# facebookresearch/momentum

Hardware: NVIDIA H100
Metric: GN iterations/sec (batched 72-joint IK) (higher is better)
Workload: dtype f32

## Files before the change

### momentum_b200/csrc/ik_chol_sched.cpp

```cpp
#include "ik_chol_sched.h"

#include "ik_chol_sched.cuh"

#include <algorithm>
#include <cstdio>
#include <cstdlib>
#include <map>
#include <set>
#include <tuple>

namespace mb2 {

namespace {

struct BitRows {
  int n, words;
  std::vector<uint64_t> b;
  BitRows(int n_) : n(n_), words((n_ + 63) / 64), b(size_t(n_) * ((n_ + 63) / 64), 0) {}
  uint64_t* row(int i) { return b.data() + size_t(i) * words; }
  const uint64_t* row(int i) const { return b.data() + size_t(i) * words; }
  void set(int i, int j) { row(i)[j >> 6] |= 1ull << (j & 63); }
  void clear(int i, int j) { row(i)[j >> 6] &= ~(1ull << (j & 63)); }
  bool test(int i, int j) const { return (row(i)[j >> 6] >> (j & 63)) & 1ull; }
  int count(int i) const {
    int c = 0;
    for (int w = 0; w < words; ++w) c += __builtin_popcountll(row(i)[w]);
    return c;
  }
};

std::vector<int> minimumDegreeOrder(BitRows& adj, const std::vector<int>* priority) {
  const int n = adj.n;
  std::vector<int> order;
  order.reserve(n);
  std::vector<uint8_t> done(n, 0);
  std::vector<int> degree(n);
  for (int i = 0; i < n; ++i) degree[i] = adj.count(i);
  int last = -1;
  for (int step = 0; step < n; ++step) {
    int best = -1;
    for (int i = 0; i < n; ++i) {
      if (done[i]) continue;
      if (best < 0 || degree[i] < degree[best]) { best = i; continue; }
      if (degree[i] != degree[best]) continue;
      const int pi = priority ? (*priority)[i] : 0, pb = priority ? (*priority)[best] : 0;
      if (pi > pb) best = i;
      else if (pi == pb && last >= 0 && adj.test(last, i) && !adj.test(last, best)) best = i;
    }
    std::vector<int> nb;
    for (int j = 0; j < n; ++j)
      if (!done[j] && j != best && adj.test(best, j)) nb.push_back(j);
    for (int u : nb) {
      uint64_t* ru = adj.row(u);
      const uint64_t* rv = adj.row(best);
      for (int w = 0; w < adj.words; ++w) ru[w] |= rv[w];
      adj.clear(u, u);
      adj.clear(u, best);
    }
    for (int u : nb) {
      int c = 0;
      for (int j : nb) c += (j != u) ? 1 : 0;
      (void)c;
      int d = 0;
      const uint64_t* ru = adj.row(u);
      for (int j = 0; j < n; ++j)
        if (!done[j] && j != best && ((ru[j >> 6] >> (j & 63)) & 1ull)) ++d;
      degree[u] = d;
    }
    done[best] = 1;
    order.push_back(best);
    last = best;
  }
  return order;
}

}

std::string buildCholSchedule(int n, const std::vector<std::vector<int>>& cliques, bool forceDense, CholSchedule& out, const std::vector<int>* priority) {
  out = CholSchedule();
  if (n <= 0) return "empty system";
  out.n = n;
  out.nParams = n;

  std::vector<int> order(n);
  BitRows pattern(n);
  for (int i = 0; i < n; ++i) pattern.set(i, i);
  if (forceDense) {
    for (int i = 0; i < n; ++i) order[i] = i;
  } else {
    for (const auto& c : cliques)
      for (int a : c) {
        if (a < 0 || a >= n) continue;
        for (int b : c)
          if (b >= 0 && b < n) pattern.set(a, b);
      }
    BitRows work = pattern;
    for (int i = 0; i < n; ++i) work.clear(i, i);
    if (priority != nullptr && int(priority->size()) != n) return "priority must have one entry per column";
    order = minimumDegreeOrder(work, priority);
  }
  std::vector<int> slot(n);
  {
    std::vector<int> rank(n);
    for (int i = 0; i < n; ++i) rank[order[i]] = i;
    BitRows F(n);
    for (int a = 0; a < n; ++a)
      for (int b = 0; b < n; ++b)
        if (a != b && (forceDense || pattern.test(a, b))) { const int i = rank[a], j = rank[b]; if (i > j) F.set(i, j); }
    std::vector<int> parent(n, -1), cnt(n, 0);
    std::vector<std::vector<int>> col(n);
    for (int j = 0; j < n; ++j) {
      for (int i = j + 1; i < n; ++i) if (F.test(i, j)) col[j].push_back(i);
      cnt[j] = int(col[j].size());
      if (!col[j].empty()) {
        const int pj = col[j][0];
        parent[j] = pj;
        for (size_t k = 1; k < col[j].size(); ++k) F.set(col[j][k], pj);
      }
    }
    int fill = 0, start = 0;
    int padded = 0;
    auto closeTile = [&]() { if (fill != 0) { padded += kCholTile - fill; fill = 0; } };
    auto flushSupernode = [&](int first, int lastExcl) {
      const int sz = lastExcl - first;
      if (sz <= kCholTile) {
        if (fill + sz > kCholTile) closeTile();
      } else {
        closeTile();
        const int head = sz % kCholTile;
        for (int j = first; j < first + head; ++j) { slot[j] = padded++; fill = (fill + 1) % kCholTile; }
        closeTile();
        first += head;
      }
      for (int j = first; j < lastExcl; ++j) { slot[j] = padded++; fill = (fill + 1) % kCholTile; }
    };
    for (int j = 1; j <= n; ++j) {
      const bool joins = j < n && parent[j - 1] == j && cnt[j - 1] == cnt[j] + 1;
      if (!joins) { flushSupernode(start, j); start = j; }
    }
    (void)fill;
    const int T0 = (padded + kCholTile - 1) / kCholTile;
    out.numTileCols = T0;
    out.nPad = T0 * kCholTile;
  }
  const int T = out.numTileCols;
  if (T > 512) return "system too large for the tile schedule";
  out.perm.assign(out.nPad, int16_t(-1));
  std::vector<int> pos(n);
  for (int i = 0; i < n; ++i) { out.perm[slot[i]] = int16_t(order[i]); pos[order[i]] = slot[i]; }

  std::vector<std::vector<uint8_t>> S(T, std::vector<uint8_t>(T, 0));
  for (int I = 0; I < T; ++I) S[I][I] = 1;
  if (forceDense) {
    for (int I = 0; I < T; ++I) for (int J = 0; J <= I; ++J) S[I][J] = 1;
  } else {
    for (int a = 0; a < n; ++a)
      for (int b = 0; b < n; ++b)
        if (pattern.test(a, b)) {
          const int I = pos[a] / kCholTile, J = pos[b] / kCholTile;
// ... 77 lines not shown
    start.assign(1, 0);
    for (int L = 0; L < numLevels; ++L) {
      std::vector<int> ids;
      for (int t = out.levelTaskStart[L]; t < out.levelTaskStart[L + 1]; ++t) ids.push_back(t);
      std::stable_sort(ids.begin(), ids.end(), [&](int a, int b) { return out.taskPairStart[a + 1] - out.taskPairStart[a] > out.taskPairStart[b + 1] - out.taskPairStart[b]; });
      std::vector<std::vector<int>> ofWarp(W);
      std::vector<int64_t> load(W, 0);
      for (int t : ids) {
        int w = 0;
        for (int k = 1; k < W; ++k) if (load[k] < load[w]) w = k;
        ofWarp[w].push_back(t);
        load[w] += 2 * (out.taskPairStart[t + 1] - out.taskPairStart[t]) + 1;
      }
      size_t rounds = 0;
      for (const auto& v : ofWarp) rounds = std::max(rounds, v.size());
      const size_t base = order.size();
      order.resize(base + rounds * W, -1);
      for (int w = 0; w < W; ++w)
        for (size_t r = 0; r < ofWarp[w].size(); ++r) order[base + r * W + w] = ofWarp[w][r];
      start.push_back(int32_t(order.size()));
    }
  }
  out.colPanelStart.assign(1, 0);
  for (int K = 0; K < T; ++K) {
    for (int I : st[K]) { out.colPanelTile.push_back(tileId[I][K]); out.colPanelRow.push_back(I); }
    out.colPanelStart.push_back(int(out.colPanelTile.size()));
  }
  for (int K = 0; K < T; ++K) { const int64_t r = T - 1 - K; out.denseTileOps += r * (r + 1) / 2; }
  out.order = order;
  if (getenv("MB2_SCHED_DUMP") != nullptr) {
    fprintf(stderr, "chol schedule: n %d nPad %d tile columns %d tiles %d levels %d tile ops %lld (dense %lld)\n", n, out.nPad, T, out.numTiles, numLevels, (long long)out.tileOps, (long long)out.denseTileOps);
    for (int L = 0; L < numLevels; ++L) {
      int maxPairs = 0, pairs = 0;
      for (int t = out.levelTaskStart[L]; t < out.levelTaskStart[L + 1]; ++t) { const int p = out.taskPairStart[t + 1] - out.taskPairStart[t]; pairs += p; maxPairs = std::max(maxPairs, p); }
      fprintf(stderr, "  level %d: %d diagonal tiles, %d panel tiles, %d update tasks (%d pairs, longest %d), %d vector tasks; columns:", L, out.levelColStart[L + 1] - out.levelColStart[L],
              out.levelPanelStart[L + 1] - out.levelPanelStart[L], out.levelTaskStart[L + 1] - out.levelTaskStart[L], pairs, maxPairs, out.levelVTaskStart[L + 1] - out.levelVTaskStart[L]);
      for (int ci = out.levelColStart[L]; ci < out.levelColStart[L + 1]; ++ci) fprintf(stderr, " %d(%d)", out.levelCols[ci], int(st[out.levelCols[ci]].size()));
      fprintf(stderr, "\n");
    }
  }
  return "";
}

std::string buildGramPlan(const CholSchedule& s, const std::vector<int32_t>& cellRow0, const std::vector<int32_t>& cellRows, const std::vector<int32_t>& cellCol,
                          int numRows, GramPlan& out) {
  out = GramPlan();
  out.numTiles = s.numTiles;
  out.numTileCols = s.numTileCols;
  const int T = s.numTileCols;
  std::map<std::pair<int, int>, int> stripId;
  for (size_t i = 0; i < cellCol.size(); ++i) {
    const int d = cellCol[i];
    if (d < 0 || d >= s.n || s.pos[d] < 0) return "Jacobian cell in a column outside the schedule";
    const int K = s.pos[d] >> 4;
    for (int q = cellRow0[i] >> 2; q <= (cellRow0[i] + cellRows[i] - 1) >> 2; ++q) stripId[{q, K}] = 0;
  }
  int next = 0;
  for (auto& kv : stripId) kv.second = next++;
  out.numStrips = next;
  out.stripCoord.resize(size_t(next) * 2);
  std::vector<std::vector<int>> ofCol(T);
  for (const auto& kv : stripId) {
    const int q = kv.first.first, K = kv.first.second;
    out.stripCoord[2 * kv.second] = 4 * q;
    out.stripCoord[2 * kv.second + 1] = s.perm[16 * K];
    ofCol[K].push_back(kv.second);
  }
  std::map<int, std::set<int>> colsOfUnit;
  std::map<int, int> rowsOfUnit;
  for (size_t i = 0; i < cellCol.size(); ++i) { colsOfUnit[cellRow0[i]].insert(s.pos[cellCol[i]] >> 4); rowsOfUnit[cellRow0[i]] = cellRows[i]; }
  std::set<std::tuple<int, int, int>> quadPairs;
  for (const auto& kv : colsOfUnit) {
    const int r0 = kv.first, r1 = r0 + rowsOfUnit[r0] - 1;
    for (int q = r0 >> 2; q <= r1 >> 2; ++q)
      for (int I : kv.second)
        for (int J : kv.second)
          if (I >= J) quadPairs.insert(std::make_tuple(q, I, J));
  }
  std::vector<std::vector<std::pair<int, int>>> pairs(s.numTiles);
  for (const auto& qp : quadPairs) {
    const int q = std::get<0>(qp), I = std::get<1>(qp), J = std::get<2>(qp);
    const int t = s.tileIdTable[size_t(I) * T + J];
    if (t < 0) return "Gram plan: a Jacobian row couples two tile columns whose tile is not in the schedule";
    pairs[t].push_back({stripId[{q, I}], stripId[{q, J}]});
  }
  out.residOff = out.numStrips * 64;
  out.stride = (out.residOff + ((numRows + 3) & ~3) + 63) / 64 * 64;
  const int zeroStrip = out.stride / 64;
  out.tilePairStart.assign(s.numTiles + 1, 0);
  for (int t = 0; t < s.numTiles; ++t) {
    out.macs += int64_t(pairs[t].size()) * 16 * 16 * 4;
    if (pairs[t].size() % 2) pairs[t].push_back({zeroStrip, zeroStrip});
    out.tilePairStart[t + 1] = out.tilePairStart[t] + int(pairs[t].size());
    for (const auto& pr : pairs[t]) { out.pairA.push_back(pr.first); out.pairB.push_back(pr.second); }
  }
  out.tileQuadStart.assign(s.numTiles + 1, 0);
  for (int t = 0; t < s.numTiles; ++t) {
    out.tileQuadStart[t + 1] = out.tileQuadStart[t] + (out.tilePairStart[t + 1] - out.tilePairStart[t]) / 2;
    for (int p = out.tilePairStart[t]; p < out.tilePairStart[t + 1]; p += 2) {
      out.quad.push_back(out.pairA[p] * 64); out.quad.push_back(out.pairB[p] * 64);
      out.quad.push_back(out.pairA[p + 1] * 64); out.quad.push_back(out.pairB[p + 1] * 64);
    }
  }
  {
    std::vector<int> byLoad(s.numTiles);
    for (int t = 0; t < s.numTiles; ++t) byLoad[t] = t;
    std::stable_sort(byLoad.begin(), byLoad.end(), [&](int a, int b) { return pairs[a].size() > pairs[b].size(); });
    std::vector<std::vector<int>> ofWarp(kGramWarps);
    std::vector<int64_t> load(kGramWarps, 0);
    for (int t : byLoad) {
      int w = 0;
      for (int k = 1; k < kGramWarps; ++k) if (load[k] < load[w]) w = k;
      ofWarp[w].push_back(t);
      load[w] += int64_t(pairs[t].size()) / 2 + 2;
    }
    size_t rounds = 0;
    for (const auto& v : ofWarp) rounds = std::max(rounds, v.size());
    out.tileOrder.assign(rounds * kGramWarps, -1);
    for (int w = 0; w < kGramWarps; ++w)
      for (size_t r = 0; r < ofWarp[w].size(); ++r) out.tileOrder[r * kGramWarps + w] = ofWarp[w][r];
  }
  std::map<int, int> stripsOfQuad;
  for (const auto& kv : stripId) ++stripsOfQuad[kv.first.first];
  out.cellStripOff.resize(cellCol.size());
  out.cellQuadStride.resize(cellCol.size());
  for (size_t i = 0; i < cellCol.size(); ++i) {
    const int d = cellCol[i], K = s.pos[d] >> 4, q0 = cellRow0[i] >> 2;
    out.cellStripOff[i] = uint32_t(stripId[{q0, K}]) * 64u + uint32_t(d - s.perm[16 * K]) * 4u;
    out.cellQuadStride[i] = uint16_t(stripsOfQuad[q0]);
    for (int q = q0 + 1; q <= (cellRow0[i] + cellRows[i] - 1) >> 2; ++q)
      if (stripsOfQuad[q] != stripsOfQuad[q0] || stripId[{q, K}] != stripId[{q0, K}] + (q - q0) * stripsOfQuad[q0]) return "Gram plan: row quads of one unit are not laid out uniformly";
  }
  out.colStripStart.assign(T + 1, 0);
  for (int K = 0; K < T; ++K) {
    out.colStripStart[K + 1] = out.colStripStart[K] + int(ofCol[K].size());
    out.colStrip.insert(out.colStrip.end(), ofCol[K].begin(), ofCol[K].end());
  }
  return "";
}

void makeGramBlob(const GramPlan& g, const CholSchedule& s, std::vector<int32_t>& blob, int32_t offsets[8]) {
  blob.clear();
  int k = 0;
  auto add = [&](const std::vector<int32_t>& v) { offsets[k++] = int32_t(blob.size()); blob.insert(blob.end(), v.begin(), v.end()); while (blob.size() % 4) blob.push_back(0); };
  add(g.tileOrder); add(g.tileQuadStart); add(g.quad); add(std::vector<int32_t>()); add(g.colStripStart); add(g.colStrip);
  std::vector<int32_t> stripRow(g.numStrips), info(s.numTiles);
  for (int i = 0; i < g.numStrips; ++i) stripRow[i] = g.stripCoord[2 * i];
  auto validOf = [&](int K) { int v = 0; while (v < kCholTile && s.perm[16 * K + v] >= 0) ++v; return v; };
  for (int t = 0; t < s.numTiles; ++t) info[t] = validOf(s.tileRow[t]) | (validOf(s.tileCol[t]) << 8) | ((s.tileRow[t] == s.tileCol[t] ? 1 : 0) << 16);
  add(stripRow); add(info);
  if (blob.empty()) blob.push_back(0);
}

std::string makeGramCholTables(const GramPlan& g, const CholSchedule& s, GramCholTables& out) {
  out = GramCholTables();
  std::vector<uint16_t>& t = out.tab;
  bool fits = true;
  auto put = [&](int64_t v) { fits = fits && v >= 0 && v <= 0xFFFF; t.push_back(uint16_t(v)); };
  auto section = [&]() { while (t.size() % 4) t.push_back(0); return int32_t(t.size()); };
  auto validOf = [&](int K) { int v = 0; while (v < kCholTile && s.perm[16 * K + v] >= 0) ++v; return v; };
  out.L.gram = section();
  for (int32_t tile : g.tileOrder) {
    if (tile < 0) { put(0xFFFF); put(0); put(0); put(0); continue; }
    fits = fits && tile < 0xFFFF;
    put(tile);
    put(validOf(s.tileRow[tile]) | (validOf(s.tileCol[tile]) << 8) | ((s.tileRow[tile] == s.tileCol[tile] ? 1 : 0) << 15));
    put(g.tileQuadStart[tile]); put(g.tileQuadStart[tile + 1]);
  }
  out.L.quad = section();
  for (int32_t v : g.quad) put(v);
  out.L.col = section();
  for (int32_t v : g.colStripStart) put(v);
  out.L.colEnt = section();
  for (int32_t sidx : g.colStrip) { put(int64_t(sidx) * 64); put(g.stripCoord[2 * sidx]); }
  out.L.level = section();
  for (int L = 0; L <= s.numLevels; ++L) { put(s.levelColStart[L]); put(s.levelPanelStart[L]); put(s.levelOrderStart8[L]); put(s.levelVTaskStart[L]); }
  out.L.diag = section();
  for (int32_t K : s.levelCols) { put(K); put(s.diagTile[K]); put(s.colPanelStart[K]); put(s.colPanelStart[K + 1]); }
  out.L.panel = section();
  for (size_t pi = 0; pi < s.panelTile.size(); ++pi) { put(s.panelTile[pi]); put(s.panelDiag[pi]); }
  out.L.order = section();
  for (int32_t ti : s.taskOrder8) {
    if (ti < 0) { put(0xFFFF); put(0); put(0); put(0); continue; }
    fits = fits && s.taskDst[ti] < 0xFFFF;
    put(s.taskDst[ti]); put(s.taskPairStart[ti]); put(s.taskPairStart[ti + 1]); put(0);
  }
  out.L.pair = section();
  for (size_t p = 0; p < s.pairA.size(); ++p) { put(s.pairA[p]); put(s.pairB[p]); }
  out.L.vtask = section();
  for (size_t vi = 0; vi < s.vtaskRow.size(); ++vi) { put(s.vtaskRow[vi]); put(s.vtaskSrcStart[vi]); put(s.vtaskSrcStart[vi + 1]); put(0); }
  out.L.vsrc = section();
  for (size_t p = 0; p < s.vsrcTile.size(); ++p) { put(s.vsrcTile[p]); put(s.vsrcCol[p]); }
  out.L.colPanel = section();
  for (size_t p = 0; p < s.colPanelTile.size(); ++p) { put(s.colPanelTile[p]); put(s.colPanelRow[p]); }
  section();
  const int64_t onStrips = (int64_t(g.stride) + 64 + 255) / 256;
  out.parkTiles = int32_t(std::min<int64_t>(s.numTiles, onStrips));
  return fits ? "" : "Gram + Cholesky tables: an entry does not fit in 16 bits";
}

void layoutDeviceColumns(CholSchedule& s, std::vector<int32_t>& deviceColumnOrder) {
  deviceColumnOrder.clear();
  s.nParams = s.n;
  for (int K = 0; K < s.numTileCols; ++K) {
    while (deviceColumnOrder.size() % 4 != 0) deviceColumnOrder.push_back(-1);
    for (int j = 0; j < kCholTile; ++j) {
      int16_t& p = s.perm[16 * K + j];
      if (p < 0) continue;
      const int dev = int(deviceColumnOrder.size());
      deviceColumnOrder.push_back(p);
      p = int16_t(dev);
    }
  }
  s.n = int32_t(deviceColumnOrder.size());
  s.pos.assign(s.n, int16_t(-1));
  for (int slot = 0; slot < s.nPad; ++slot) if (s.perm[slot] >= 0) s.pos[s.perm[slot]] = int16_t(slot);
  s.order.assign(deviceColumnOrder.begin(), deviceColumnOrder.end());
}

}

namespace mb2 {

void makeScheduleBlob(const CholSchedule& s, std::vector<int32_t>& blob, CholSchedDev& dev) {
  blob.clear();
  std::vector<size_t> offs;
  auto add16 = [&](const std::vector<int16_t>& v) { offs.push_back(blob.size()); for (int16_t x : v) blob.push_back(int32_t(x)); while (blob.size() % 4) blob.push_back(0); };
  auto add32 = [&](const std::vector<int32_t>& v) { offs.push_back(blob.size()); blob.insert(blob.end(), v.begin(), v.end()); while (blob.size() % 4) blob.push_back(0); };
  add16(s.perm); add16(s.pos); add16(s.tileIdTable); add16(s.tileRow); add16(s.tileCol);
  add32(s.diagTile); add32(s.levelColStart); add32(s.levelCols); add32(s.levelPanelStart); add32(s.panelTile); add32(s.panelDiag);
  add32(s.levelTaskStart); add32(s.taskDst); add32(s.taskPairStart); add32(s.pairA); add32(s.pairB); add32(s.levelVTaskStart); add32(s.vtaskRow);
  add32(s.vtaskSrcStart); add32(s.vsrcTile); add32(s.vsrcCol); add32(s.colPanelStart); add32(s.colPanelTile); add32(s.colPanelRow);
  add32(s.levelOrderStart8); add32(s.taskOrder8); add32(s.levelOrderStart16); add32(s.taskOrder16);
  {
    std::vector<int32_t> info(size_t(s.numTiles) * 3, 0);
    auto validOf = [&](int K) { int v = 0; while (v < kCholTile && s.perm[16 * K + v] >= 0) ++v; return v; };
    for (int t = 0; t < s.numTiles; ++t) {
      const int I = s.tileRow[t], J = s.tileCol[t];
      const int vI = validOf(I), vJ = validOf(J);
      info[3 * t] = vI > 0 ? s.perm[16 * I] : 0;
      info[3 * t + 1] = vJ > 0 ? s.perm[16 * J] : 0;
      info[3 * t + 2] = vI | (vJ << 8) | ((I == J ? 1 : 0) << 16);
    }
    add32(info);
  }
  if (blob.empty()) blob.push_back(0);
  dev = CholSchedDev();
  dev.n = s.n; dev.nPad = s.nPad; dev.numTileCols = s.numTileCols; dev.numTiles = s.numTiles; dev.numLevels = s.numLevels;
  const int32_t* b = blob.data();
  dev.blob = b;
  dev.blobInts = int32_t(blob.size());
  int k = 0;
  dev.perm = b + offs[k++]; dev.pos = b + offs[k++]; dev.tileIdTable = b + offs[k++]; dev.tileRow = b + offs[k++]; dev.tileCol = b + offs[k++];
  dev.diagTile = b + offs[k++]; dev.levelColStart = b + offs[k++]; dev.levelCols = b + offs[k++]; dev.levelPanelStart = b + offs[k++];
  dev.panelTile = b + offs[k++]; dev.panelDiag = b + offs[k++]; dev.levelTaskStart = b + offs[k++]; dev.taskDst = b + offs[k++];
  dev.taskPairStart = b + offs[k++]; dev.pairA = b + offs[k++]; dev.pairB = b + offs[k++]; dev.levelVTaskStart = b + offs[k++]; dev.vtaskRow = b + offs[k++];
  dev.vtaskSrcStart = b + offs[k++]; dev.vsrcTile = b + offs[k++]; dev.vsrcCol = b + offs[k++]; dev.colPanelStart = b + offs[k++];
  dev.colPanelTile = b + offs[k++]; dev.colPanelRow = b + offs[k++];
  dev.levelOrderStart8 = b + offs[k++]; dev.taskOrder8 = b + offs[k++]; dev.levelOrderStart16 = b + offs[k++]; dev.taskOrder16 = b + offs[k++];
  dev.tileInfo = b + offs[k++];
}

}
```

### momentum_b200/csrc/ik_chol_sched.h

```cpp
#pragma once

#include <cstdint>
#include <string>
#include <vector>

namespace mb2 {

constexpr int kCholTile = 16;

struct CholSchedule {
  int32_t n{0}, nPad{0}, numTileCols{0}, numTiles{0}, numLevels{0};
  int32_t nParams{0};
  std::vector<int16_t> perm;
  std::vector<int16_t> pos;
  std::vector<int16_t> tileIdTable;
  std::vector<int16_t> tileRow, tileCol;
  std::vector<int32_t> diagTile;
  std::vector<int32_t> levelColStart, levelCols;
  std::vector<int32_t> levelPanelStart, panelTile, panelDiag, panelRow;
  std::vector<int32_t> levelTaskStart, taskDst, taskPairStart, pairA, pairB;
  std::vector<int32_t> levelOrderStart8, taskOrder8, levelOrderStart16, taskOrder16;
  std::vector<int32_t> levelVTaskStart, vtaskRow, vtaskSrcStart, vsrcTile, vsrcCol;
  std::vector<int32_t> colPanelStart, colPanelTile, colPanelRow;
  std::vector<int> order;
  int64_t tileOps{0};
  int64_t denseTileOps{0};
};

std::string buildCholSchedule(int n, const std::vector<std::vector<int>>& cliques, bool forceDense, CholSchedule& out, const std::vector<int>* priority = nullptr);
void layoutDeviceColumns(CholSchedule& s, std::vector<int32_t>& deviceColumnOrder);

inline int cholSchedLdH(int n) { return (n + 1 + 15) / 16 * 16; }
constexpr int kGramWarps = 8;
constexpr int kGramCholMaxRounds = 8;
struct GramPlan {
  int32_t numStrips{0}, numTiles{0}, numTileCols{0};
  std::vector<int32_t> stripCoord;
  std::vector<int32_t> tileOrder;
  std::vector<int32_t> tilePairStart;
  std::vector<int32_t> pairA, pairB;
  std::vector<int32_t> tileQuadStart;
  std::vector<int32_t> quad;
  std::vector<int32_t> colStripStart;
  std::vector<int32_t> colStrip;
  std::vector<uint32_t> cellStripOff;
  std::vector<uint16_t> cellQuadStride;
  int32_t residOff{0};
  int32_t stride{0};
  int64_t macs{0};
};
std::string buildGramPlan(const CholSchedule& s, const std::vector<int32_t>& cellRow0, const std::vector<int32_t>& cellRows, const std::vector<int32_t>& cellCol,
                          int numRows, GramPlan& out);

void makeGramBlob(const GramPlan& g, const CholSchedule& s, std::vector<int32_t>& blob, int32_t offsets[8]);

struct CholSchedDev;
void makeScheduleBlob(const CholSchedule& s, std::vector<int32_t>& blob, CholSchedDev& dev);

struct GramCholLayout {
  int32_t gram, quad, col, colEnt, level, diag, panel, order, pair, vtask, vsrc, colPanel;
};
struct GramCholTables {
  GramCholLayout L{};
  std::vector<uint16_t> tab;
  int32_t parkTiles{0};
};
std::string makeGramCholTables(const GramPlan& g, const CholSchedule& s, GramCholTables& out);

}
```

### momentum_b200/csrc/ik_kernels.cu

```cuda
#include "ik_kernels.cuh"

#include <algorithm>
#include <cstdio>
#include <type_traits>

#include "ik_chol.cuh"
#include "ik_chol_sched.h"
#include "ik_jtj_tc.cuh"
#include "ik_ptx.cuh"
#include "ik_device.cuh"
#include "ik_jacobi.cuh"

namespace mb2 {

__device__ __forceinline__ double warpSum(double v) {
  for (int o = 16; o > 0; o >>= 1) v += __shfl_xor_sync(0xffffffffu, v, o);
  return v;
}

size_t sweepSmemPerInstance(const FunctionTables& T, int warpsPerInstance) {
  const size_t nPad = (T.numParams + 3) & ~3;
  const size_t jp = warpsPerInstance > 1 ? size_t((T.numJoints * kParametersPerJoint + 1) & ~1) : 0;
  return sizeof(float) * (nPad + jp + size_t((T.numJoints * kJointStateStride + 1) & ~1) + size_t((T.recStride + 1) & ~1) + 4 + 2 * size_t(warpsPerInstance));
}
// ... 1889 lines not shown
        bulkLoad(smemAddr(tiles) + off, reinterpret_cast<const char*>(src) + off, total - off < 16384u ? total - off : 16384u, barAddr);
    }
  } else {
    if (tid == 0) {
      bulkLoad(smemAddr(blob), Sg.blob, blobBytes, barAddr);
      bulkLoad(smemAddr(gsub), a.g + size_t(b) * a.ldG, gBytes, barAddr);
    }
    for (int t = tid; t < Sg.numTiles; t += kSchedThreads) {
      const int gi0 = __ldg(Sg.tileInfo + 3 * t), gj0 = __ldg(Sg.tileInfo + 3 * t + 1);
      tmaLoad3d(smemAddr(tiles + size_t(t) * 256), &hmap, gi0, gj0, b, barAddr);
    }
  }
  MB2_PROF(6)
  mbarWaitRelaxed(barAddr, 0);
  MB2_PROF(7)
  const CholSchedDev S = rebaseSchedule(Sg, blob);
  if (fromGram) {
    for (int s = tid; s < S.nPad; s += kSchedThreads) {
      const int p = S.perm[s];
      if (p >= 0) gsub[p] = y[s];
    }
  } else {
    for (int t = warp; t < S.numTiles; t += kSchedThreads / 32) cholConvertBox(tiles + size_t(t) * 256, S.tileInfo[3 * t + 2], lane);
    for (int s = tid; s < S.nPad; s += kSchedThreads) {
      const int p = S.perm[s];
      y[s] = p >= 0 ? gsub[p] : 0.f;
    }
  }
  __syncthreads();
  MB2_PROF(8)
  if (!fromGram)
    for (int s = tid; s < S.nPad; s += kSchedThreads)
      if (S.perm[s] >= 0) tiles[size_t(S.diagTile[s >> 4]) * 256 + tileIdx(s & 15, s & 15)] += a.regularization;
  __syncthreads();
  MB2_PROF(0)

  for (int L = 0; L < S.numLevels; ++L) {
    for (int ci = S.levelColStart[L] + warp; ci < S.levelColStart[L + 1]; ci += kSchedThreads / 32) {
      const int K = S.levelCols[ci];
      cholDiagTile(tiles + size_t(S.diagTile[K]) * 256, y + 16 * K, lane, a.regularization, flags);
    }
    __syncthreads();
    MB2_PROF(1)
    for (int pi = S.levelPanelStart[L] + warp; pi < S.levelPanelStart[L + 1]; pi += kSchedThreads / 32) {
      float* ptile = tiles + size_t(S.panelTile[pi]) * 256;
      float x[2][4];
      cholPanelProduct(ptile, tiles + size_t(S.panelDiag[pi]) * 256, lane, x);
      cholPanelStore(ptile, lane, x);
    }
    __syncthreads();
    MB2_PROF(2)
    {
      const int32_t* oStart = kSchedThreads == 256 ? S.levelOrderStart8 : S.levelOrderStart16, *order = kSchedThreads == 256 ? S.taskOrder8 : S.taskOrder16;
      for (int oi = oStart[L] + warp; oi < oStart[L + 1]; oi += kSchedThreads / 32) { const int ti = order[oi]; if (ti >= 0) cholUpdateTask(tiles, S, ti, lane); }
    }
    for (int vi = S.levelVTaskStart[L] + hw; vi < S.levelVTaskStart[L + 1]; vi += kSchedThreads / 16) cholVectorTask(tiles, y, S, vi, hl);
    __syncthreads();
    MB2_PROF(3)
  }
  for (int L = S.numLevels - 1; L >= 0; --L) {
    for (int ci = S.levelColStart[L] + warp; ci < S.levelColStart[L + 1]; ci += kSchedThreads / 32) cholBackwardColumn(tiles, y, S, S.levelCols[ci], lane);
    __syncthreads();
  }
  MB2_PROF(4)
  for (int i = tid; i < S.nPad; i += kSchedThreads) { const int p = S.perm[i]; if (p >= 0) dsub[p] = y[i]; }
  __syncthreads();
  cholFinish(a, b, n, dsub, gsub, flags[0] != 0);
  MB2_PROF(5)
  if (kProfile && b == 0 && tid == 0)
    printf("chol-profile (cycles, block 0): blob %lld issue %lld wait %lld lambda %lld diag %lld panel %lld update %lld backward %lld finish %lld | levels %d tiles %d\n", pc[6], pc[7],
           pc[8], pc[0], pc[1], pc[2], pc[3], pc[4], pc[5], S.numLevels, S.numTiles);
#undef MB2_PROF
}

cudaError_t launchCholeskyScheduled(const CholArgs& a, const CholSchedDev& sched, int threads, cudaStream_t stream) {
  const size_t smem = choleskyScheduledSmemBytes(a.ns, sched.nPad, sched.numTiles, sched.blobInts);
  if (smem > size_t(g_maxSmemOptin) || (threads != 256 && threads != 512)) return cudaErrorInvalidConfiguration;
  const bool wide = threads == 512;
  const bool prof = (a.profile & 1) != 0;
  cudaError_t e;
  if (wide) e = prof ? cudaFuncSetAttribute(choleskyScheduledKernel<512, true>, cudaFuncAttributeMaxDynamicSharedMemorySize, int(smem))
                     : cudaFuncSetAttribute(choleskyScheduledKernel<512, false>, cudaFuncAttributeMaxDynamicSharedMemorySize, int(smem));
  else e = prof ? cudaFuncSetAttribute(choleskyScheduledKernel<256, true>, cudaFuncAttributeMaxDynamicSharedMemorySize, int(smem))
                : cudaFuncSetAttribute(choleskyScheduledKernel<256, false>, cudaFuncAttributeMaxDynamicSharedMemorySize, int(smem));
  if (e != cudaSuccess) return e;
  if (a.tilesIn == nullptr && (a.g == nullptr || a.ldG != cholGradientLd(a.ns))) return cudaErrorInvalidValue;
  if ((a.ldH & 3) != 0 || (a.hStride & 3) != 0 || (a.tilesStride & 3) != 0) return cudaErrorInvalidValue;
  CUtensorMap hmap;
  const bool fromGram = a.tilesIn != nullptr;
  const uint64_t dims[3] = {uint64_t(fromGram ? 256 : a.ldH), uint64_t(fromGram ? sched.numTiles : a.ns + 1), uint64_t(a.batch)};
  const uint64_t strides[2] = {uint64_t(fromGram ? 256 : a.ldH) * sizeof(float), uint64_t(fromGram ? a.tilesStride : a.hStride) * sizeof(float)};
  const uint32_t box[3] = {16u, 16u, 1u};
  e = makeTensorMap3d(&hmap, fromGram ? a.tilesIn : a.H, dims, strides, box, 64);
  if (e != cudaSuccess) return e;
  if (wide && prof) choleskyScheduledKernel<512, true><<<a.batch, 512, smem, stream>>>(hmap, a, sched);
  else if (wide) choleskyScheduledKernel<512, false><<<a.batch, 512, smem, stream>>>(hmap, a, sched);
  else if (prof) choleskyScheduledKernel<256, true><<<a.batch, 256, smem, stream>>>(hmap, a, sched);
  else choleskyScheduledKernel<256, false><<<a.batch, 256, smem, stream>>>(hmap, a, sched);
  return cudaGetLastError();
}

__device__ int acquireParkSlot(uint32_t* words, int numWords, int start) {
  for (int w = start % numWords;; w = (w + 1 == numWords) ? 0 : w + 1) {
    uint32_t freeBits = ~__ldcg(words + w);
    while (freeBits != 0u) {
      const int bit = __ffs(freeBits) - 1;
      if ((atomicOr(words + w, 1u << bit) & (1u << bit)) == 0u) return 32 * w + bit;
      freeBits &= freeBits - 1u;
    }
  }
}

template <bool kProfile, class Tables>
__global__ void __launch_bounds__(kGramThreads, 4) gramCholeskyKernel(const GramCholArgs a, const CholSchedDev S, const __grid_constant__ Tables P) {
  extern __shared__ __align__(16) float gcSmem[];
  const GramArgs& g = a.g;
  const CholArgs& c = a.c;
  const int b = blockIdx.x;
  if (c.active[b] == 0) return;
  const int n = c.ns, tid = threadIdx.x;
  const int warp = tid >> 5, lane = tid & 31, hw = tid >> 4, hl = tid & 15;
  constexpr int kWarps = kGramThreads / 32;
  float* U = gcSmem + (((128u - (smemAddr(gcSmem) & 127u)) & 127u) >> 2);
  const size_t tileFloats = size_t(S.numTiles) * 256, sweepFloats = g.stripStride + 64;
  const size_t uni = ((tileFloats > sweepFloats ? tileFloats : sweepFloats) + 3) & ~size_t(3);
  float* strips = U;
  float* resid = U + g.residOff;
  float* tiles = U;
  float* y = U + uni;
  float* gsub = y + S.nPad;
  int* flags = reinterpret_cast<int*>(gsub + ((n + 3) & ~3));
  unsigned long long* bar = reinterpret_cast<unsigned long long*>(flags + 4);
  const uint16_t* tab = P.tab;
  const GramCholLayout& L = P.L;
  long long pc[8] = {0, 0, 0, 0, 0, 0, 0, 0}, pt = 0;
  if constexpr (kProfile) pt = clock64();
#define MB2_GC(k) if constexpr (kProfile) { const long long now = clock64(); pc[k] += now - pt; pt = now; }
  const uint32_t barAddr = smemAddr(bar);
  const uint32_t stripBytes = uint32_t(g.stripStride) * 4u;
  if (tid == 0) {
    flags[0] = 0;
    mbarInit(barAddr, 1);
    fenceBarrierInit();
    mbarExpectTx(barAddr, stripBytes);
    const char* src = reinterpret_cast<const char*>(g.strips + size_t(b) * g.stripStride);
    for (uint32_t off = 0; off < stripBytes; off += 16384u) bulkLoad(smemAddr(strips) + off, src + off, stripBytes - off < 16384u ? stripBytes - off : 16384u, barAddr);
    flags[1] = a.parkTiles > 0 ? acquireParkSlot(a.parkSlots, a.parkSlotWords, b) : 0;
  }
  if (tid >= 64 && tid < 128) strips[g.stripStride + (tid - 64)] = 0.f;
  __syncthreads();
  mbarWaitRelaxed(barAddr, 0);
  MB2_GC(0)
  float* park = a.park + size_t(flags[1]) * size_t(a.parkTiles) * 256 + 4 * lane;
  const int rounds = g.numOrder / kWarps;
  auto tileInfoOf = [](int packed) { return (packed & 0x7FFF) | ((packed >> 15) << 16); };
  for (int r = 0; r < rounds; ++r) {
    const int4 rec = tableRecord4(tab + L.gram + 4 * (r * kWarps + warp));
    if (rec.x == 0xFFFF) continue;
    float acc[2][4];
#pragma unroll
    for (int i = 0; i < 2; ++i)
#pragma unroll
      for (int j = 0; j < 4; ++j) acc[i][j] = 0.f;
    gramTileAccumulate(strips, tab + L.quad, rec.z, rec.w, lane, acc);
    if (rec.x >= a.parkTiles) gramTileStore(tiles + size_t(rec.x) * 256, acc, tileInfoOf(rec.y), g.regularization, lane);
    else {
      __stcg(reinterpret_cast<float4*>(park + size_t(rec.x) * 256), make_float4(acc[0][0], acc[0][1], acc[0][2], acc[0][3]));
      __stcg(reinterpret_cast<float4*>(park + size_t(rec.x) * 256 + 128), make_float4(acc[1][0], acc[1][1], acc[1][2], acc[1][3]));
    }
  }
  for (int K = hw; K < S.numTileCols; K += kGramThreads / 16)
    y[16 * K + hl] = gramVectorEntry(strips, resid, tab + L.colEnt, int(tab[L.col + K]), int(tab[L.col + K + 1]), hl);
  __syncthreads();
  MB2_GC(1)
  for (int r = 0; r < rounds; ++r) {
    const int4 rec = tableRecord4(tab + L.gram + 4 * (r * kWarps + warp));
    if (rec.x == 0xFFFF || rec.x >= a.parkTiles) continue;
    const float4 v0 = __ldcg(reinterpret_cast<const float4*>(park + size_t(rec.x) * 256));
    const float4 v1 = __ldcg(reinterpret_cast<const float4*>(park + size_t(rec.x) * 256 + 128));
    const float acc[2][4] = {{v0.x, v0.y, v0.z, v0.w}, {v1.x, v1.y, v1.z, v1.w}};
    gramTileStore(tiles + size_t(rec.x) * 256, acc, tileInfoOf(rec.y), g.regularization, lane);
  }
  for (int s2 = tid; s2 < S.nPad; s2 += kGramThreads) {
    const int p = S.perm[s2];
    if (p >= 0) gsub[p] = y[s2];
  }
  __syncthreads();
  if (tid == 0 && a.parkTiles > 0) atomicAnd(a.parkSlots + (flags[1] >> 5), ~(1u << (flags[1] & 31)));
  MB2_GC(2)
  for (int Lv = 0; Lv < S.numLevels; ++Lv) {
    const int4 l0 = tableRecord4(tab + L.level + 4 * Lv), l1 = tableRecord4(tab + L.level + 4 * (Lv + 1));
    for (int ci = l0.x + warp; ci < l1.x; ci += kWarps) {
      const int4 d = tableRecord4(tab + L.diag + 4 * ci);
      cholDiagTile(tiles + size_t(d.y) * 256, y + 16 * d.x, lane, c.regularization, flags);
    }
    __syncthreads();
    MB2_GC(3)
    for (int pi = l0.y + warp; pi < l1.y; pi += kWarps) {
      const int2 pe = tableRecord2(tab + L.panel + 2 * pi);
      float* ptile = tiles + size_t(pe.x) * 256;
      float x[2][4];
      cholPanelProduct(ptile, tiles + size_t(pe.y) * 256, lane, x);
      cholPanelStore(ptile, lane, x);
    }
    __syncthreads();
    MB2_GC(4)
    for (int oi = l0.z + warp; oi < l1.z; oi += kWarps) {
      const int4 o = tableRecord4(tab + L.order + 4 * oi);
      if (o.x != 0xFFFF) cholUpdateTile(tiles, tab + L.pair, tab + L.pair + 1, 2, o.y, o.z, o.x, lane);
    }
    for (int vi = l0.w + hw; vi < l1.w; vi += kGramThreads / 16) {
      const int4 v = tableRecord4(tab + L.vtask + 4 * vi);
      cholVectorRows(tiles, y, tab + L.vsrc, tab + L.vsrc + 1, 2, v.y, v.z, v.x, hl);
    }
    __syncthreads();
    MB2_GC(5)
  }
  for (int Lv = S.numLevels - 1; Lv >= 0; --Lv) {
    const int c0 = tab[L.level + 4 * Lv], c1 = tab[L.level + 4 * (Lv + 1)];
    for (int ci = c0 + warp; ci < c1; ci += kWarps) {
      const int4 d = tableRecord4(tab + L.diag + 4 * ci);
      cholBackwardPanels(tiles, y, tab + L.colPanel, tab + L.colPanel + 1, 2, d.z, d.w, d.x, d.y, lane);
    }
    __syncthreads();
  }
  MB2_GC(6)
  cholFinish(c, b, n, y, gsub, flags[0] != 0, S.pos);
  MB2_GC(7)
  if constexpr (kProfile) {
    if (b == int(gridDim.x >> 1) && tid == 0 && a.phaseCycles != nullptr)
      for (int k = 0; k < 8; ++k) a.phaseCycles[k] += (unsigned long long)pc[k];
  }
#undef MB2_GC
}

template <bool kProfile, class Tables>
static cudaError_t prepareGramCholesky(size_t smem) {
  cudaError_t e = cudaFuncSetAttribute(gramCholeskyKernel<kProfile, Tables>, cudaFuncAttributeMaxDynamicSharedMemorySize, int(smem));
  if (e != cudaSuccess) return e;
  return cudaFuncSetAttribute(gramCholeskyKernel<kProfile, Tables>, cudaFuncAttributePreferredSharedMemoryCarveout, int(cudaSharedmemCarveoutMaxShared));
}

int gramCholeskyParkSlots(const GramCholArgs& a, const CholSchedDev& sched, bool paramTables) {
  const size_t smem = gramCholeskySmemBytes(a.g.stripStride, a.c.ns, sched.nPad, sched.numTiles);
  cudaError_t e = paramTables ? prepareGramCholesky<false, GramCholParamTables>(smem) : prepareGramCholesky<false, GramCholGlobalTables>(smem);
  int perSm = 0;
  if (e == cudaSuccess)
    e = paramTables ? cudaOccupancyMaxActiveBlocksPerMultiprocessor(&perSm, gramCholeskyKernel<false, GramCholParamTables>, kGramThreads, smem)
                    : cudaOccupancyMaxActiveBlocksPerMultiprocessor(&perSm, gramCholeskyKernel<false, GramCholGlobalTables>, kGramThreads, smem);
  if (e != cudaSuccess || perSm < 1) return -1;
  return (g_numSms * perSm + 31) / 32 * 32;
}

cudaError_t launchGramCholesky(const GramCholArgs& a, const CholSchedDev& sched, const GramCholParamTables* inParams, const GramCholGlobalTables& inGlobal, bool profile,
                               cudaStream_t stream) {
  const size_t smem = gramCholeskySmemBytes(a.g.stripStride, a.c.ns, sched.nPad, sched.numTiles);
  if (smem > size_t(g_maxSmemOptin) || (a.g.stripStride & 3) != 0) return cudaErrorInvalidConfiguration;
  if (a.parkTiles > 0 && (a.park == nullptr || a.parkSlots == nullptr || a.parkSlotWords < 1)) return cudaErrorInvalidValue;
  cudaError_t e;
  if (inParams != nullptr) e = profile ? prepareGramCholesky<true, GramCholParamTables>(smem) : prepareGramCholesky<false, GramCholParamTables>(smem);
  else e = profile ? prepareGramCholesky<true, GramCholGlobalTables>(smem) : prepareGramCholesky<false, GramCholGlobalTables>(smem);
  if (e != cudaSuccess) return e;
  if (inParams != nullptr) {
    if (profile) gramCholeskyKernel<true, GramCholParamTables><<<a.c.batch, kGramThreads, smem, stream>>>(a, sched, *inParams);
    else gramCholeskyKernel<false, GramCholParamTables><<<a.c.batch, kGramThreads, smem, stream>>>(a, sched, *inParams);
  } else {
    if (profile) gramCholeskyKernel<true, GramCholGlobalTables><<<a.c.batch, kGramThreads, smem, stream>>>(a, sched, inGlobal);
    else gramCholeskyKernel<false, GramCholGlobalTables><<<a.c.batch, kGramThreads, smem, stream>>>(a, sched, inGlobal);
  }
  return cudaGetLastError();
}

}
#include "ik_qr.cuh"
#include "ik_tr_qr.cuh"
namespace mb2 {

cudaError_t initKernelAttributes() {
  int dev = 0;
  cudaError_t e = cudaGetDevice(&dev);
  if (e != cudaSuccess) return e;
  e = cudaDeviceGetAttribute(&g_numSms, cudaDevAttrMultiProcessorCount, dev);
  if (e != cudaSuccess) return e;
  e = cudaDeviceGetAttribute(&g_maxSmemPerSm, cudaDevAttrMaxSharedMemoryPerMultiprocessor, dev);
  if (e != cudaSuccess) return e;
  return cudaDeviceGetAttribute(&g_maxSmemOptin, cudaDevAttrMaxSharedMemoryPerBlockOptin, dev);
}

__global__ void trialUpdateKernel(int batch, const float* thetaOrig, int ldTheta, const float* delta, int ns, const int32_t* cols, const float* scale,
                                  float* thetaTrial, const int32_t* active) {
  const int b = blockIdx.x;
  if (active[b] == 0) return;
  const float s = scale[b];
  for (int i = threadIdx.x; i < ns; i += blockDim.x) {
    const int c = cols[i];
    if (c >= 0) thetaTrial[size_t(b) * ldTheta + c] = thetaOrig[size_t(b) * ldTheta + c] - s * delta[size_t(b) * ns + i];
  }
}
cudaError_t launchTrialUpdate(int batch, const float* thetaOrig, int ldTheta, const float* delta, int ns, const int32_t* cols, const float* scale,
                              float* thetaTrial, const int32_t* active, cudaStream_t stream) {
  trialUpdateKernel<<<batch, 128, 0, stream>>>(batch, thetaOrig, ldTheta, delta, ns, cols, scale, thetaTrial, active);
  return cudaGetLastError();
}

__global__ void lineSearchStepKernel(const LineSearchArgs a) {
  const int b = blockIdx.x * blockDim.x + threadIdx.x;
  if (b >= a.batch || a.searching[b] == 0) return;
  const double error = a.errors[b], errorNew = a.trialErrors[b];
  const float scale = a.scale[b];
  bool accept;
  if (!a.subsetVariant) {
    const float scaledError = 1e-3f * (float)error;
    accept = (error - errorNew) >= (double)(scale * scaledError);
  } else {
    accept = (error - errorNew) >= (double)(1e-4f * scale) * (double)a.gradDotDelta[b];
  }
  if (accept || a.step >= 9) a.searching[b] = 0;
  else a.scale[b] = scale * 0.5f;
}
cudaError_t launchLineSearchStep(const LineSearchArgs& a, cudaStream_t stream) {
  lineSearchStepKernel<<<(a.batch + 127) / 128, 128, 0, stream>>>(a);
  return cudaGetLastError();
}

__global__ void commitTrialKernel(int batch, int numParams, int ldTheta, const float* thetaTrial, float* theta, const int32_t* active) {
  const int b = blockIdx.x;
  if (active[b] == 0) return;
  for (int i = threadIdx.x; i < numParams; i += blockDim.x) theta[size_t(b) * ldTheta + i] = thetaTrial[size_t(b) * ldTheta + i];
}
cudaError_t launchCommitTrial(int batch, int numParams, int ldTheta, const float* thetaTrial, float* theta, const int32_t* active, cudaStream_t stream) {
  commitTrialKernel<<<batch, 128, 0, stream>>>(batch, numParams, ldTheta, thetaTrial, theta, active);
  return cudaGetLastError();
}

// ... 46 lines not shown
```

Measured before the change: 9.578 million.

## Schedule Gram tiles in epochs with slot remapping to avoid global parking

Adds a host-side search that groups Gram tiles into epochs and remaps tile storage slots, so tiles whose shared-memory slot overlaps the live strip data are written only after their readers finish. One tile per warp is held in registers across the epoch barrier, which removes the round trip through global park memory. Cholesky tables are rewritten to use the remapped slots. The cost is extra __syncthreads between epochs and a bounded combinatorial search at setup, with a fallback to the old parking path when no placement is found.

```diff
diff --git a/momentum_b200/csrc/ik_chol_sched.cpp b/momentum_b200/csrc/ik_chol_sched.cpp
--- a/momentum_b200/csrc/ik_chol_sched.cpp
+++ b/momentum_b200/csrc/ik_chol_sched.cpp
@@ -5,6 +5,7 @@
 #include <algorithm>
 #include <cstdio>
 #include <cstdlib>
+#include <functional>
 #include <map>
 #include <set>
 #include <tuple>
@@ -388,6 +389,151 @@
   if (blob.empty()) blob.push_back(0);
 }
 
+namespace {
+
+struct GramTilePlacement {
+  std::vector<int32_t> order;
+  std::vector<uint8_t> held;
+  std::vector<int32_t> epochEnd;
+  std::vector<int32_t> slotOf;
+};
+
+constexpr int kGramMaxEpochs = 4;
+constexpr int kGramPlacementNodes = 20000;
+
+int64_t dealTiles(const std::vector<int>& tiles, const std::vector<int64_t>& cost, std::vector<std::vector<int>>& ofWarp) {
+  std::vector<int> byLoad(tiles);
+  std::stable_sort(byLoad.begin(), byLoad.end(), [&](int a, int b) { return cost[a] > cost[b]; });
+  ofWarp.assign(kGramWarps, std::vector<int>());
+  std::vector<int64_t> load(kGramWarps, 0);
+  for (int t : byLoad) {
+    int w = 0;
+    for (int k = 1; k < kGramWarps; ++k) if (load[k] < load[w]) w = k;
+    ofWarp[w].push_back(t);
+    load[w] += cost[t];
+  }
+  return *std::max_element(load.begin(), load.end());
+}
+
+bool placeGramTiles(const GramPlan& g, int numTiles, GramTilePlacement& out) {
+  const int N = numTiles;
+  std::vector<int64_t> cost(N);
+  std::vector<std::vector<int>> readers(N);
+  for (int t = 0; t < N; ++t) {
+    cost[t] = int64_t(g.tileQuadStart[t + 1] - g.tileQuadStart[t]) + 2;
+    for (int q = g.tileQuadStart[t]; q < g.tileQuadStart[t + 1]; ++q)
+      for (int k = 0; k < 4; ++k) {
+        const int slot = g.quad[4 * q + k] / 256;
+        if (slot < N && (readers[slot].empty() || readers[slot].back() != t)) readers[slot].push_back(t);
+      }
+  }
+  std::vector<uint8_t> jtr(N, 0);
+  for (int k = 0; k < N && int64_t(k) * 256 < g.stride; ++k) jtr[k] = 1;
+  std::vector<int> epochOf(N, -1);
+  auto deadAfter = [&](int k, int e) {
+    if (jtr[k] && e < 0) return false;
+    for (int t : readers[k]) if (epochOf[t] < 0 || epochOf[t] > e) return false;
+    return true;
+  };
+  int freeSlots = 0;
+  for (int k = 0; k < N; ++k) freeSlots += deadAfter(k, -1) ? 1 : 0;
+  int64_t best = -1;
+  std::vector<int> bestEpoch;
+  int nodes = 0;
+  std::vector<std::vector<int>> ofWarp;
+  std::function<void(int, int, int, int64_t)> search = [&](int e, int freeNow, int remaining, int64_t total) {
+    if (++nodes > kGramPlacementNodes || (best >= 0 && total >= best)) return;
+    std::vector<int> rest;
+    for (int t = 0; t < N; ++t) if (epochOf[t] < 0) rest.push_back(t);
+    const int held = std::min(kGramWarps, remaining);
+    if (remaining - held <= freeNow) {
+      const int64_t tot = total + dealTiles(rest, cost, ofWarp);
+      if (best < 0 || tot < best) { best = tot; bestEpoch = epochOf; for (int t : rest) bestEpoch[t] = e; }
+      return;
+    }
+    if (e + 1 >= kGramMaxEpochs) return;
+    const int cap = freeNow + kGramWarps;
+    std::vector<uint8_t> in(N, 0);
+    int taken = 0;
+    for (;;) {
+      int bestSlot = -1, bestNeed = 0;
+      for (int k = 0; k < N; ++k) {
+        if (deadAfter(k, e - 1)) continue;
+        int need = 0;
+        for (int t : readers[k]) need += (epochOf[t] < 0 && !in[t]) ? 1 : 0;
+        if (need == 0 || taken + need > cap) continue;
+        if (bestSlot < 0 || need < bestNeed) { bestSlot = k; bestNeed = need; }
+      }
+      if (bestSlot < 0) break;
+      for (int t : readers[bestSlot]) if (epochOf[t] < 0 && !in[t]) { in[t] = 1; ++taken; }
+    }
+    std::vector<int> fill;
+    for (int t : rest) if (!in[t]) fill.push_back(t);
+    std::stable_sort(fill.begin(), fill.end(), [&](int a, int b) { return cost[a] > cost[b]; });
+    for (int extra = 0; extra <= int(fill.size()) && taken + extra <= cap; ++extra) {
+      std::vector<int> S;
+      for (int t : rest) if (in[t]) S.push_back(t);
+      S.insert(S.end(), fill.begin(), fill.begin() + extra);
+      if (S.empty()) continue;
+      const int64_t span = dealTiles(S, cost, ofWarp);
+      int h = 0;
+      for (const auto& v : ofWarp) h += v.empty() ? 0 : 1;
+      const int direct = int(S.size()) - h;
+      if (direct > freeNow) continue;
+      int before = 0, after = 0;
+      for (int k = 0; k < N; ++k) before += deadAfter(k, e - 1) ? 1 : 0;
+      for (int t : S) epochOf[t] = e;
+      for (int k = 0; k < N; ++k) after += deadAfter(k, e) ? 1 : 0;
+      const int freeNext = freeNow - direct + (after - before) - h;
+      if (freeNext >= 0) search(e + 1, freeNext, remaining - int(S.size()), total + span + 1);
+      for (int t : S) epochOf[t] = -1;
+    }
+  };
+  search(0, freeSlots, N, 0);
+  if (best < 0) return false;
+  epochOf = bestEpoch;
+  const int numEpochs = 1 + *std::max_element(epochOf.begin(), epochOf.end());
+  out = GramTilePlacement();
+  std::vector<int> ready(N);
+  for (int e = 0; e < numEpochs; ++e) {
+    std::vector<int> S;
+    for (int t = 0; t < N; ++t) if (epochOf[t] == e) S.push_back(t);
+    dealTiles(S, cost, ofWarp);
+    size_t rounds = 0;
+    for (const auto& v : ofWarp) rounds = std::max(rounds, v.size());
+    const size_t base = out.order.size();
+    out.order.resize(base + rounds * kGramWarps, -1);
+    out.held.resize(out.order.size(), 0);
+    for (int w = 0; w < kGramWarps; ++w)
+      for (size_t r = 0; r < ofWarp[w].size(); ++r) {
+        const int t = ofWarp[w][r];
+        const bool last = r + 1 == ofWarp[w].size();
+        out.order[base + r * kGramWarps + w] = t;
+        out.held[base + r * kGramWarps + w] = last ? 1 : 0;
+        ready[t] = last ? e + 1 : e;
+      }
+    out.epochEnd.push_back(int32_t(out.order.size() / kGramWarps));
+  }
+  std::vector<int> dead(N, 0);
+  for (int k = 0; k < N; ++k) {
+    dead[k] = jtr[k] ? 1 : 0;
+    for (int t : readers[k]) dead[k] = std::max(dead[k], epochOf[t] + 1);
+  }
+  std::vector<int> byReady(N);
+  for (int t = 0; t < N; ++t) byReady[t] = t;
+  std::stable_sort(byReady.begin(), byReady.end(), [&](int a, int b) { return ready[a] < ready[b]; });
+  std::vector<uint8_t> used(N, 0);
+  out.slotOf.assign(N, -1);
+  for (int t : byReady) {
+    for (int k = 0; k < N; ++k)
+      if (!used[k] && dead[k] <= ready[t]) { used[k] = 1; out.slotOf[t] = k; break; }
+    if (out.slotOf[t] < 0) return false;
+  }
+  return true;
+}
+
+}
+
 std::string makeGramCholTables(const GramPlan& g, const CholSchedule& s, GramCholTables& out) {
   out = GramCholTables();
   std::vector<uint16_t>& t = out.tab;
@@ -395,12 +541,26 @@
   auto put = [&](int64_t v) { fits = fits && v >= 0 && v <= 0xFFFF; t.push_back(uint16_t(v)); };
   auto section = [&]() { while (t.size() % 4) t.push_back(0); return int32_t(t.size()); };
   auto validOf = [&](int K) { int v = 0; while (v < kCholTile && s.perm[16 * K + v] >= 0) ++v; return v; };
+  GramTilePlacement pl;
+  const bool placed = placeGramTiles(g, s.numTiles, pl);
+  if (!placed) {
+    pl.order = g.tileOrder;
+    pl.held.assign(pl.order.size(), 0);
+    pl.epochEnd.assign(1, int32_t(pl.order.size() / kGramWarps));
+    pl.slotOf.resize(s.numTiles);
+    for (int k = 0; k < s.numTiles; ++k) pl.slotOf[k] = k;
+  }
+  out.slotOf = pl.slotOf;
+  const std::vector<int32_t>& slot = pl.slotOf;
+  std::vector<int32_t> epochEnd = pl.epochEnd;
   out.L.gram = section();
-  for (int32_t tile : g.tileOrder) {
+  for (size_t i = 0; i < pl.order.size(); ++i) {
+    const int32_t tile = pl.order[i];
     if (tile < 0) { put(0xFFFF); put(0); put(0); put(0); continue; }
-    fits = fits && tile < 0xFFFF;
-    put(tile);
-    put(validOf(s.tileRow[tile]) | (validOf(s.tileCol[tile]) << 8) | ((s.tileRow[tile] == s.tileCol[tile] ? 1 : 0) << 15));
+    fits = fits && slot[tile] < 0xFFFF;
+    out.heldTiles += pl.held[i];
+    put(slot[tile]);
+    put(validOf(s.tileRow[tile]) | (validOf(s.tileCol[tile]) << 8) | (int(pl.held[i]) << 14) | ((s.tileRow[tile] == s.tileCol[tile] ? 1 : 0) << 15));
     put(g.tileQuadStart[tile]); put(g.tileQuadStart[tile + 1]);
   }
   out.L.quad = section();
@@ -412,26 +572,30 @@
   out.L.level = section();
   for (int L = 0; L <= s.numLevels; ++L) { put(s.levelColStart[L]); put(s.levelPanelStart[L]); put(s.levelOrderStart8[L]); put(s.levelVTaskStart[L]); }
   out.L.diag = section();
-  for (int32_t K : s.levelCols) { put(K); put(s.diagTile[K]); put(s.colPanelStart[K]); put(s.colPanelStart[K + 1]); }
+  for (int32_t K : s.levelCols) { put(K); put(slot[s.diagTile[K]]); put(s.colPanelStart[K]); put(s.colPanelStart[K + 1]); }
   out.L.panel = section();
-  for (size_t pi = 0; pi < s.panelTile.size(); ++pi) { put(s.panelTile[pi]); put(s.panelDiag[pi]); }
+  for (size_t pi = 0; pi < s.panelTile.size(); ++pi) { put(slot[s.panelTile[pi]]); put(slot[s.panelDiag[pi]]); }
   out.L.order = section();
   for (int32_t ti : s.taskOrder8) {
     if (ti < 0) { put(0xFFFF); put(0); put(0); put(0); continue; }
-    fits = fits && s.taskDst[ti] < 0xFFFF;
-    put(s.taskDst[ti]); put(s.taskPairStart[ti]); put(s.taskPairStart[ti + 1]); put(0);
+    fits = fits && slot[s.taskDst[ti]] < 0xFFFF;
+    put(slot[s.taskDst[ti]]); put(s.taskPairStart[ti]); put(s.taskPairStart[ti + 1]); put(0);
   }
   out.L.pair = section();
-  for (size_t p = 0; p < s.pairA.size(); ++p) { put(s.pairA[p]); put(s.pairB[p]); }
+  for (size_t p = 0; p < s.pairA.size(); ++p) { put(slot[s.pairA[p]]); put(slot[s.pairB[p]]); }
   out.L.vtask = section();
   for (size_t vi = 0; vi < s.vtaskRow.size(); ++vi) { put(s.vtaskRow[vi]); put(s.vtaskSrcStart[vi]); put(s.vtaskSrcStart[vi + 1]); put(0); }
   out.L.vsrc = section();
-  for (size_t p = 0; p < s.vsrcTile.size(); ++p) { put(s.vsrcTile[p]); put(s.vsrcCol[p]); }
+  for (size_t p = 0; p < s.vsrcTile.size(); ++p) { put(slot[s.vsrcTile[p]]); put(s.vsrcCol[p]); }
   out.L.colPanel = section();
-  for (size_t p = 0; p < s.colPanelTile.size(); ++p) { put(s.colPanelTile[p]); put(s.colPanelRow[p]); }
+  for (size_t p = 0; p < s.colPanelTile.size(); ++p) { put(slot[s.colPanelTile[p]]); put(s.colPanelRow[p]); }
+  out.L.epoch = section();
+  put(int64_t(epochEnd.size()));
+  put(0);
+  for (int r : epochEnd) put(r);
   section();
-  const int64_t onStrips = (int64_t(g.stride) + 64 + 255) / 256;
-  out.parkTiles = int32_t(std::min<int64_t>(s.numTiles, onStrips));
+  out.epochs = int32_t(epochEnd.size());
+  out.parkTiles = placed ? 0 : int32_t(std::min<int64_t>(s.numTiles, (int64_t(g.stride) + 64 + 255) / 256));
   return fits ? "" : "Gram + Cholesky tables: an entry does not fit in 16 bits";
 }
 
diff --git a/momentum_b200/csrc/ik_chol_sched.h b/momentum_b200/csrc/ik_chol_sched.h
--- a/momentum_b200/csrc/ik_chol_sched.h
+++ b/momentum_b200/csrc/ik_chol_sched.h
@@ -58,12 +58,15 @@
 void makeScheduleBlob(const CholSchedule& s, std::vector<int32_t>& blob, CholSchedDev& dev);
 
 struct GramCholLayout {
-  int32_t gram, quad, col, colEnt, level, diag, panel, order, pair, vtask, vsrc, colPanel;
+  int32_t gram, quad, col, colEnt, level, diag, panel, order, pair, vtask, vsrc, colPanel, epoch;
 };
 struct GramCholTables {
   GramCholLayout L{};
   std::vector<uint16_t> tab;
   int32_t parkTiles{0};
+  int32_t epochs{1};
+  int32_t heldTiles{0};
+  std::vector<int32_t> slotOf;
 };
 std::string makeGramCholTables(const GramPlan& g, const CholSchedule& s, GramCholTables& out);
 
diff --git a/momentum_b200/csrc/ik_kernels.cu b/momentum_b200/csrc/ik_kernels.cu
--- a/momentum_b200/csrc/ik_kernels.cu
+++ b/momentum_b200/csrc/ik_kernels.cu
@@ -2065,34 +2065,43 @@
   mbarWaitRelaxed(barAddr, 0);
   MB2_GC(0)
   float* park = a.park + size_t(flags[1]) * size_t(a.parkTiles) * 256 + 4 * lane;
-  const int rounds = g.numOrder / kWarps;
-  auto tileInfoOf = [](int packed) { return (packed & 0x7FFF) | ((packed >> 15) << 16); };
-  for (int r = 0; r < rounds; ++r) {
-    const int4 rec = tableRecord4(tab + L.gram + 4 * (r * kWarps + warp));
-    if (rec.x == 0xFFFF) continue;
+  auto tileInfoOf = [](int packed) { return (packed & 0x3FFF) | ((packed >> 15) << 16); };
+  const int epochs = tab[L.epoch];
+  for (int e = 0, r = 0; e < epochs; ++e) {
+    const int rEnd = tab[L.epoch + 2 + e];
     float acc[2][4];
-#pragma unroll
-    for (int i = 0; i < 2; ++i)
-#pragma unroll
-      for (int j = 0; j < 4; ++j) acc[i][j] = 0.f;
-    gramTileAccumulate(strips, tab + L.quad, rec.z, rec.w, lane, acc);
-    if (rec.x >= a.parkTiles) gramTileStore(tiles + size_t(rec.x) * 256, acc, tileInfoOf(rec.y), g.regularization, lane);
-    else {
-      __stcg(reinterpret_cast<float4*>(park + size_t(rec.x) * 256), make_float4(acc[0][0], acc[0][1], acc[0][2], acc[0][3]));
-      __stcg(reinterpret_cast<float4*>(park + size_t(rec.x) * 256 + 128), make_float4(acc[1][0], acc[1][1], acc[1][2], acc[1][3]));
-    }
-  }
-  for (int K = hw; K < S.numTileCols; K += kGramThreads / 16)
-    y[16 * K + hl] = gramVectorEntry(strips, resid, tab + L.colEnt, int(tab[L.col + K]), int(tab[L.col + K + 1]), hl);
-  __syncthreads();
+    int held = 0xFFFF, heldInfo = 0;
+    for (; r < rEnd; ++r) {
+      const int4 rec = tableRecord4(tab + L.gram + 4 * (r * kWarps + warp));
+      if (rec.x == 0xFFFF) continue;
+#pragma unroll
+      for (int i = 0; i < 2; ++i)
+#pragma unroll
+        for (int j = 0; j < 4; ++j) acc[i][j] = 0.f;
+      gramTileAccumulate(strips, tab + L.quad, rec.z, rec.w, lane, acc);
+      if (rec.y & 0x4000) { held = rec.x; heldInfo = rec.y; }
+      else if (rec.x >= a.parkTiles) gramTileStore(tiles + size_t(rec.x) * 256, acc, tileInfoOf(rec.y), g.regularization, lane);
+      else {
+        __stcg(reinterpret_cast<float4*>(park + size_t(rec.x) * 256), make_float4(acc[0][0], acc[0][1], acc[0][2], acc[0][3]));
+        __stcg(reinterpret_cast<float4*>(park + size_t(rec.x) * 256 + 128), make_float4(acc[1][0], acc[1][1], acc[1][2], acc[1][3]));
+      }
+    }
+    if (e == 0)
+      for (int K = hw; K < S.numTileCols; K += kGramThreads / 16)
+        y[16 * K + hl] = gramVectorEntry(strips, resid, tab + L.colEnt, int(tab[L.col + K]), int(tab[L.col + K + 1]), hl);
+    __syncthreads();
+    if (held != 0xFFFF) gramTileStore(tiles + size_t(held) * 256, acc, tileInfoOf(heldInfo), g.regularization, lane);
+  }
   MB2_GC(1)
-  for (int r = 0; r < rounds; ++r) {
-    const int4 rec = tableRecord4(tab + L.gram + 4 * (r * kWarps + warp));
-    if (rec.x == 0xFFFF || rec.x >= a.parkTiles) continue;
-    const float4 v0 = __ldcg(reinterpret_cast<const float4*>(park + size_t(rec.x) * 256));
-    const float4 v1 = __ldcg(reinterpret_cast<const float4*>(park + size_t(rec.x) * 256 + 128));
-    const float acc[2][4] = {{v0.x, v0.y, v0.z, v0.w}, {v1.x, v1.y, v1.z, v1.w}};
-    gramTileStore(tiles + size_t(rec.x) * 256, acc, tileInfoOf(rec.y), g.regularization, lane);
+  if (a.parkTiles > 0) {
+    for (int r = 0; r < tab[L.epoch + 2]; ++r) {
+      const int4 rec = tableRecord4(tab + L.gram + 4 * (r * kWarps + warp));
+      if (rec.x == 0xFFFF || rec.x >= a.parkTiles) continue;
+      const float4 v0 = __ldcg(reinterpret_cast<const float4*>(park + size_t(rec.x) * 256));
+      const float4 v1 = __ldcg(reinterpret_cast<const float4*>(park + size_t(rec.x) * 256 + 128));
+      const float acc[2][4] = {{v0.x, v0.y, v0.z, v0.w}, {v1.x, v1.y, v1.z, v1.w}};
+      gramTileStore(tiles + size_t(rec.x) * 256, acc, tileInfoOf(rec.y), g.regularization, lane);
+    }
   }
   for (int s2 = tid; s2 < S.nPad; s2 += kGramThreads) {
     const int p = S.perm[s2];
```

Result: no change. 9.672 million, median of 6 (+1.0%).
